# holandes22/etcd

Hardware: AMD Instinct MI355X
Metric: MsgAppResp applied/sec + commits advanced/sec, 1M raft groups×3, 1-8 GPUs (higher is better)
Workload: dtype u64

## Files before the change

etcd_amd/csrc/hipbatch.hip:

```cpp
#include <hip/hip_runtime.h>

#include <algorithm>
#include <cstdio>
#include <cstdlib>
#include <cstring>
#include <type_traits>
#include <utility>
#include <vector>

#include "hbmem.h"
#include "hipbatch_kernels.h"
#include "hipbatch_fast.h"
#include "hipbatch_elect.h"
#include "hipbatch_lead.h"
#include "hipbatch_wire.h"
#include "hipbatch_wire_in.h"
#include "hipbatch_wire_out.h"
#include "hipbatch_bin.h"

using namespace hb;

#define HB_CHECK(expr)                                                       \
  do {                                                                       \
    hipError_t _e = (expr);                                                  \
// ... 2777 lines not shown
  }
  if (threadIdx.x == 0) {
    a.bbase[nblk] = tot;
    decf_finish(a, tot);
  }
}
__global__ void __launch_bounds__(DEC_THREADS) k_decf_write(DecfArgs a, uint32_t nblk) {
  decf_write_block(a, blockIdx.x, a.bbase[blockIdx.x], a.bbase[nblk] <= a.ent_cap);
}
__global__ void __launch_bounds__(DEC_THREADS) k_decf_small(DecfArgs a, uint32_t nblk) {
  __shared__ uint64_t sh16[16];
  __shared__ uint64_t l_base[DEC_THREADS];
  uint64_t tot;
  l_base[threadIdx.x] = block_excl_scan64(threadIdx.x < nblk ? (uint64_t)a.bsum[threadIdx.x] : 0ull, sh16, &tot);
  __syncthreads();
  if (threadIdx.x == 0) decf_finish(a, tot);
  for (uint32_t b = 0; b < nblk; ++b) decf_write_block(a, b, l_base[b], tot <= a.ent_cap);
}

__global__ void __launch_bounds__(128) k_finish(uint64_t* shard, uint64_t* stats, uint64_t* accum) {
  const int map[ST_N + 1] = {HB_STAT_MSGS,  HB_STAT_APPRESP, HB_STAT_VOTERESP, HB_STAT_DROPPED, HB_STAT_COMMITS,
                             HB_STAT_WON,   HB_STAT_LOST,    HB_STAT_FAULTS,   HB_STAT_ENTRIES, HB_STAT_EVENTS};
  const uint32_t t = threadIdx.x, k = t / NSH;
  uint64_t v = 0;
  if (k <= ST_N) {
    v = shard[shard_at(k, t % NSH)];
    shard[shard_at(k, t % NSH)] = 0;
  }
#pragma unroll
  for (uint32_t d = 1; d < NSH; d <<= 1) v += __shfl_xor(v, d);
  if (k <= ST_N && t % NSH == 0) {
    stats[map[k]] = v;
    if (accum) accum[map[k]] += v;
  }
}

__global__ void k_load(DevState S, uint32_t first, uint32_t count, const hb_group* src) {
  const uint32_t i = blockIdx.x * blockDim.x + threadIdx.x;
  if (i >= count) return;
  const uint32_t g = first + i;
  const hb_group& r = src[i];
  S.term[g] = r.term;
  S.commit[g] = r.committed;
  S.first[g] = r.first_index;
  S.last[g] = r.last_index;
  S.tfirst[g] = r.term_first;
  S.tlast[g] = r.term_last;
  S.snap[g] = r.snap_index;
  uint64_t m = meta_make(r.state, r.n, r.self_slot, r.lead, r.vote, r.fault, r.votes_resp, r.votes_grant);
  if (r.term_last == r.last_index) m |= M_TL;
  if (r.self_slot < r.n && r.pr[r.self_slot].match == r.last_index && r.pr[r.self_slot].next == r.last_index + 1)
    m |= M_SM;
  if (r.commit_zero && r.committed != 0) m |= M_NC;
  S.meta[g] = m;
  S.elapsed[g] = 0;
  S.rpos[g] = 0;
  if (S.szx) {
    S.szlo[g] = r.last_index;
    *cum_at(S.szx[g], r.last_index) = 0;
  }
  S.trc[g] = 0;
  for (uint32_t s = 0; s < S.nmax; ++s) {
    const bool on = s < r.n;
    const size_t o = (size_t)s * S.G + g;
    S.match[o] = on ? r.pr[s].match : 0;
    S.next[o] = on ? r.pr[s].next : 0;
    S.pending[o] = on ? r.pr[s].pending_snapshot : 0;
    S.pm[o] = on ? pm_make(r.pr[s].state, r.pr[s].paused, r.pr[s].ins_start, r.pr[s].ins_count) : 0;
  }
}

__global__ void k_gather(DevState S, uint32_t first, uint32_t count, hb_group* dst) {
  const uint32_t i = blockIdx.x * blockDim.x + threadIdx.x;
  if (i >= count) return;
  const uint32_t g = first + i;
  hb_group r;
  memset(&r, 0, sizeof(r));
  const uint64_t m = S.meta[g];
  r.term = S.term[g];
  r.committed = S.commit[g];
  r.first_index = S.first[g];
  r.last_index = S.last[g];
  r.term_first = S.tfirst[g];
  r.term_last = (m & M_TL) ? r.last_index : S.tlast[g];
  r.snap_index = S.snap[g];
  r.state = m_state(m);
  r.n = m_n(m);
  r.self_slot = m_self(m);
  r.lead = m_lead(m);
  r.vote = m_vote(m);
  r.fault = m_fault(m);
  r.votes_resp = m_resp(m);
  r.votes_grant = m_grant(m);
  r.commit_zero = (m & M_NC) ? 1u : 0u;
  for (uint32_t s = 0; s < S.nmax && s < r.n; ++s) {
    const size_t o = (size_t)s * S.G + g;
    uint32_t p = S.pm[o];
    const bool kept = !((m & M_SM) && s == r.self_slot);
    r.pr[s].match = kept ? S.match[o] : r.last_index;
    r.pr[s].next = kept ? S.next[o] : r.last_index + 1;
    if (m & M_RS) rs_progress(m, s, r.last_index, r.term_first, &r.pr[s].match, &r.pr[s].next, &p);
    r.pr[s].state = pm_state(p);
    r.pr[s].paused = pm_paused(p);
    r.pr[s].ins_start = pm_start(p);
    r.pr[s].ins_count = pm_count(p);
    r.pr[s].pending_snapshot = pm_state(p) == HB_PR_SNAPSHOT ? S.pending[o] : 0;
  }
  dst[i] = r;
}

__global__ void k_set_bounds(DevState S, uint32_t count, const uint32_t* groups, const uint64_t* first,
                             const uint64_t* snap) {
  const uint32_t i = blockIdx.x * blockDim.x + threadIdx.x;
  if (i >= count) return;
  const uint32_t g = groups[i];
  S.first[g] = first[i];
  S.snap[g] = snap[i];
}

__global__ void k_load_runs(DevState S, uint32_t count, const uint32_t* groups, const uint32_t* n_runs,
                            const uint64_t* off, const uint64_t* runs) {
  const uint32_t i = blockIdx.x * blockDim.x + threadIdx.x;
  if (i >= count) return;
  const uint32_t g = groups[i], k = n_runs[i];
  uint64_t* R = lx_base(S.trx[g]);
  for (uint32_t j = 0; j < k; ++j) {
    R[2 * j] = runs[2 * (off[i] + j)];
    R[2 * j + 1] = runs[2 * (off[i] + j) + 1];
  }
  S.trc[g] = k;
}

__global__ void k_load_sizes(DevState S, uint32_t count, const uint32_t* groups, const uint32_t* n_sizes,
                             const uint64_t* off, const uint32_t* sizes) {
  const uint32_t i = blockIdx.x * blockDim.x + threadIdx.x;
  if (i >= count) return;
  const uint32_t g = groups[i], k = n_sizes[i];
  const uint64_t last = S.last[g], lo = last - k, x = S.szx[g];
  const uint32_t* z = sizes + off[i];
  uint64_t acc = 0;
  *cum_at(x, lo) = 0;
  for (uint32_t j = 1; j <= k; ++j) {
    acc += z[j - 1];
    *cum_at(x, lo + j) = acc;
  }
  S.szlo[g] = lo;
}

__global__ void k_regrow(DevState S, uint32_t count, const uint64_t* jobs) {
  const uint32_t i = blockIdx.x * blockDim.x + threadIdx.x;
  if (i >= count) return;
  const uint64_t* j = jobs + 4 * (size_t)i;
  const uint32_t g = (uint32_t)j[0], kind = (uint32_t)(j[0] >> 32);
  const uint64_t ox = j[1], nx = j[2];
  if (kind == 0) {
    const uint64_t lo = S.szlo[g], last = S.last[g];
    for (uint64_t k = lo; k <= last; ++k) *cum_at(nx, k) = *cum_at(ox, k);
    S.szx[g] = nx;
  } else {
    const uint64_t c = S.trc[g];
    const uint32_t n = (uint32_t)c, h = (uint32_t)(c >> 32);
// ... 1539 lines not shown
    const uint32_t gg = std::min(lists, GEN_GRID3 ? std::min(grid, GEN_GRID3) : grid);
    hipLaunchKernelGGL(k_apply<NMAX>, dim3(gg), dim3(PART), 0, h->stream, a);
  } else {
    hipLaunchKernelGGL(k_apply<NMAX>, dim3(std::min(lists, GEN_GRID ? std::min(grid, GEN_GRID) : grid)), dim3(PART), 0,
                       h->stream, a);
    hipLaunchKernelGGL(k_follow<NMAX>, dim3(FOLLOW_GRID), dim3(PART), 0, h->stream, a);
  }
  if (ev && full) (void)hipEventRecord(ev[4], h->stream);
}

}

extern "C" {

int hb_abi_version(void) { return HB_ABI_VERSION; }

const char* hb_strerror(int code) {
  switch (code) {
    case HB_OK: return "ok";
    case HB_EINVAL: return "invalid argument";
    case HB_ENOMEM: return "out of memory";
    case HB_EDEVICE: return "device error";
    case HB_EINVARIANT: return "device invariant violated";
    default: return "unknown error";
  }
}

int hb_create(int device, uint32_t capacity, uint32_t max_replicas, uint32_t max_inflight,
              uint64_t max_msg_size, uint64_t max_batch, hb_handle** out) {
  if (!out || capacity == 0 || max_replicas < 1 || max_replicas > HB_MAX_REPLICAS || max_inflight < 1 ||
      max_inflight > HB_MAX_INFLIGHT || max_batch >= (1ull << 31) || capacity > (1u << 24))
    return HB_EINVAL;
  int ndev = 0;
  if (hipGetDeviceCount(&ndev) != hipSuccess || device < 0 || device >= ndev) return HB_EDEVICE;
  DeviceGuard guard(device);
  hb_handle* h = new hb_handle();
  h->device = device;
  h->G = capacity;
  h->nmax = max_replicas <= 3 ? 3 : (max_replicas <= 5 ? 5 : 7);
  h->W = max_inflight;
  h->max_msg_size = max_msg_size;
  h->max_batch = max_batch;
  h->NB = (capacity + PART - 1) / PART;
  if (const char* e = getenv("HB_SMALL_STEP")) h->no_small = e[0] == '0';
  if (const char* e = getenv("HB_ROUTE_FUSE")) h->fuse = (uint32_t)atoi(e);
  if (const char* e = getenv("HB_STORM")) h->storm = atoi(e) == 0 ? 0u : 2u;
  if (const char* e = getenv("HB_FAST_STEADY")) h->steady = atoi(e) != 0;
  if (const char* e = getenv("HB_FAST_STEADY_COUNT")) h->steady_count = atoi(e) != 0;
  const size_t G = capacity, R = h->nmax;
  DevState& s = h->st;
  s.G = capacity;
  s.W = max_inflight;
  s.nmax = h->nmax;
  s.max_msg_size = max_msg_size;
  int rc = HB_OK;
#define ALLOC(ptr, count) \
  if (rc == HB_OK) rc = dalloc_t(h, &(ptr), (count))
  ALLOC(s.term, G);
  ALLOC(s.commit, G);
  ALLOC(s.first, G);
  ALLOC(s.last, G);
  ALLOC(s.tfirst, G);
  ALLOC(s.tlast, G);
  ALLOC(s.snap, G);
  ALLOC(s.meta, G);
  ALLOC(s.match, R * G);
  ALLOC(s.next, R * G);
  ALLOC(s.pending, R * G);
  ALLOC(s.pm, R * G);
  ALLOC(s.ring, R * (size_t)max_inflight * G);
  ALLOC(s.elapsed, G);
  ALLOC(s.rpos, G);
  ALLOC(s.tcfg, G);
  ALLOC(s.trx, G);
  ALLOC(s.trc, G);
  if (sz_on(max_msg_size)) {
    ALLOC(s.szx, G);
    ALLOC(s.szlo, G);
  }
  const size_t mb = max_batch ? max_batch : 1;
  auto nbk_for = [&](uint32_t sl) { return (capacity + (PART << sl) - 1) / (PART << sl); };
  auto passes_for = [&](uint32_t sl) {
    return (std::max<uint32_t>(ceil_log2(nbk_for(sl)), 1) + RDX_BITS - 1) / RDX_BITS;
  };
  const uint32_t sl_max = h->nmax <= 3 ? SIS_LOG_MAX3 : SIS_LOG_MAX;
  h->sis_log = sl_max;
  const uint32_t sl_min = route_rg_log(route_kmax(h->nmax)) - PART_LOG;
  while (h->sis_log > sl_min && passes_for(h->sis_log - 1) == passes_for(sl_max)) --h->sis_log;
  if (const char* e = getenv("HB_SIS_LOG")) {
    const int v = atoi(e);
    if (v >= (int)sl_min && v <= (int)sl_max) h->sis_log = (uint32_t)v;
  }
  h->NBK = nbk_for(h->sis_log);
  h->passes = passes_for(h->sis_log);
  h->bk_bits = std::max<uint32_t>(ceil_log2(h->NBK), 1);
  h->agrid = apply_grid_for(h->NBK, h->sis_log, h->NB);
  const size_t tiles_max = (mb + RDX_TILE - 1) / RDX_TILE;
  ALLOC(h->hist, (size_t)RDX_BINS * tiles_max);
  ALLOC(h->n_valid, 4);
  ALLOC(h->totals, RDX_BINS);
  if (h->passes == 1) {
    const size_t nhw = (tiles_max + HIST_TPB - 1) / HIST_TPB;
    h->sup_max = (uint32_t)((nhw + SB_HW - 1) / SB_HW);
    ALLOC(h->hagg, nhw * RDX_BINS);
    ALLOC(h->hsup, (size_t)SUP_BUFS * h->sup_max * RDX_BINS);
    if (rc == HB_OK && hipMemset(h->hsup, 0, (size_t)SUP_BUFS * h->sup_max * RDX_BINS * 4) != hipSuccess)
// ... 1284 lines not shown
int hb_stats_device(hb_handle* h, uint64_t** dev_stats) {
  if (!h || !dev_stats) return HB_EINVAL;
  *dev_stats = h->stats;
  return HB_OK;
}

int hb_stats(hb_handle* h, uint64_t* out) {
  if (!h || !out) return HB_EINVAL;
  DeviceGuard guard(h->device);
  HB_CHECK(hipMemcpyAsync(out, h->stats, HB_STAT_COUNT * 8, hipMemcpyDeviceToHost, h->stream));
  HB_CHECK(hipStreamSynchronize(h->stream));
  return HB_OK;
}

int hb_phase_ms(hb_handle* h, float* out, uint32_t* steps) {
  if (!h || !out) return HB_EINVAL;
  DeviceGuard guard(h->device);
  const uint32_t n = std::min<uint32_t>(h->prof_n, hb_handle::PROF_RING);
  if (steps) *steps = n;
  for (int i = 0; i < HB_PHASE_COUNT; ++i) out[i] = 0.f;
  if (n == 0) return HB_EINVAL;
  HB_CHECK(hipStreamSynchronize(h->prep));
  HB_CHECK(hipStreamSynchronize(h->stream));
  static const int span[HB_PHASE_COUNT][2] = {{0, 1}, {2, 3}, {3, 4}, {4, 5}};
  uint32_t nfull = 0;
  for (uint32_t k = 0; k < n; ++k) nfull += h->prof_full[k] ? 1u : 0u;
  for (uint32_t k = 0; k < n; ++k) {
    for (int i = 0; i < HB_PHASE_COUNT; ++i) {
      if (i != HB_PHASE_APPLY && !h->prof_full[k]) continue;
      float ms = 0.f;
      HB_CHECK(hipEventElapsedTime(&ms, h->ph[k][span[i][0]], h->ph[k][span[i][1]]));
      out[i] += ms / (float)(i == HB_PHASE_APPLY ? n : nfull);
    }
  }
  return HB_OK;
}

int hb_step_kernels(hb_handle* h, uint32_t* mask) {
  if (!h || !mask) return HB_EINVAL;
  *mask = h->kern;
  return HB_OK;
}

int hb_steady_waves(hb_handle* h, uint32_t* n) {
  if (!h || !n) return HB_EINVAL;
  *n = 0;
  if (!h->stepped || !h->steady_count) return HB_OK;
  DeviceGuard guard(h->device);
  HB_CHECK(hipStreamSynchronize(h->stream));
  HB_CHECK(hipMemcpy(n, h->set[h->cur].ctr + CTR_STEADY, 4, hipMemcpyDeviceToHost));
  return HB_OK;
}

int hb_phase_reset(hb_handle* h) {
  if (!h) return HB_EINVAL;
  h->prof_n = 0;
  return HB_OK;
}

int hb_set_stats_accum(hb_handle* h, uint64_t* dev_accum) {
  if (!h) return HB_EINVAL;
  h->stats_accum = dev_accum;
  return HB_OK;
}

int hb_set_input_stream(hb_handle* h, void* stream) {
  if (!h) return HB_EINVAL;
  h->in_stream = reinterpret_cast<hipStream_t>(stream);
  h->in_stream_set = true;
  return HB_OK;
}

int hb_stats_to(hb_handle* h, uint64_t* dev_dst) {
  if (!h || !dev_dst) return HB_EINVAL;
  DeviceGuard guard(h->device);
  HB_CHECK(hipMemcpyAsync(dev_dst, h->stats, HB_STAT_COUNT * 8, hipMemcpyDeviceToDevice, h->stream));
  return HB_OK;
}

int hb_alloc_pinned(size_t bytes, void** out) {
  if (!out) return HB_EINVAL;
  return hipHostMalloc(out, bytes ? bytes : 1, hipHostMallocDefault) == hipSuccess ? HB_OK : HB_ENOMEM;
}

int hb_free_pinned(void* p) { return hipHostFree(p) == hipSuccess ? HB_OK : HB_EDEVICE; }

}
```

etcd_amd/csrc/hipbatch_elect.h:

```cpp
#pragma once

#include "hipbatch_kernels.h"

namespace hb {

template <int NMAX>
struct ElectLane {
  DevState S;
  EvSink E;
  uint32_t g;
  uint64_t term, committed, last, tfirst, tlast, meta, meta0;
  uint64_t rlast;
  uint32_t dirty;
  uint32_t won, lost, nev;
  bool rst;
  bool sent;

  __device__ __forceinline__ uint32_t n() const { return m_n(meta); }
  __device__ __forceinline__ uint32_t state() const { return m_state(meta); }
  __device__ __forceinline__ uint32_t self() const { return m_self(meta); }
  __device__ __forceinline__ uint32_t lead() const { return m_lead(meta); }
  __device__ __forceinline__ uint32_t vote() const { return m_vote(meta); }
  __device__ __forceinline__ uint64_t soft() const {
    return (uint64_t)state() | ((uint64_t)lead() << 8) | ((uint64_t)vote() << 16);
  }
  __device__ __forceinline__ void set_field(int shift, uint64_t mask, uint64_t v) {
    meta = (meta & ~(mask << shift)) | ((v & mask) << shift);
    dirty |= D_META;
  }
  __device__ __forceinline__ void set_state(uint32_t v) { set_field(0, 3, v); }
  __device__ __forceinline__ void set_lead(uint32_t v) { set_field(9, 0xF, v); }
  __device__ __forceinline__ void set_vote(uint32_t v) { set_field(13, 0xF, v); }
  __device__ __forceinline__ void set_votes(uint32_t resp, uint32_t grant) {
    set_field(M_RESP_SHIFT, 0xFF, resp);
    set_field(M_GRANT_SHIFT, 0xFF, grant);
  }
  __device__ __forceinline__ void ev(uint32_t type, uint32_t to, uint32_t aux, uint64_t x) {
    emit_ev(E, g & (PART - 1), type, to, aux, x);
    nev++;
  }

  __device__ __forceinline__ void load() {
    term = S.term[g];
    committed = S.commit[g];
    last = S.last[g];
    tfirst = S.tfirst[g];
    tlast = S.tlast[g];
    meta0 = meta;
    if (meta & M_TL) tlast = last;
    dirty = 0;
    won = lost = nev = 0;
    rst = sent = false;
    rlast = 0;
  }

  __device__ __forceinline__ void store() {
    const uint32_t sf = self(), nn = n();
    const bool tl = tlast == last;
    const bool sm = rst ? sf < nn : (meta0 & M_SM) != 0;
    const bool leader = state() == HB_STATE_LEADER;
    const bool rs = rst && (leader ? (tfirst == rlast + 1 && (sent || nn <= 1)) : (rlast == last && !sent));
    const uint64_t m2 = (meta & ~(M_TL | M_SM | M_RS)) | (tl ? M_TL : 0ull) | (sm ? M_SM : 0ull) |
                        (rs ? M_RS : (rst ? 0ull : (meta & M_RS)));
    if (m2 != meta) {
      meta = m2;
      dirty |= D_META;
    }
    if (!tl && (meta0 & M_TL)) dirty |= D_TRUN;
    if (dirty & D_META) S.meta[g] = meta;
    if (dirty & D_TERM) S.term[g] = term;
    if (dirty & D_COMMIT) S.commit[g] = committed;
    if (dirty & D_LAST) S.last[g] = last;
    if (dirty & D_TRUN) {
      S.tfirst[g] = tfirst;
      S.tlast[g] = tlast;
    }
    if (dirty & D_ELAPSED) S.elapsed[g] = 0;
    if (rst && !rs) {
      const uint32_t peer_pm = pm_make(HB_PR_PROBE, sent ? 1u : 0u, 0, 0);
#pragma unroll
      for (int s = 0; s < NMAX; ++s) {
        if ((uint32_t)s < nn) {
          const bool me = (uint32_t)s == sf;
          S.match[(size_t)s * S.G + g] = me ? last : 0ull;
          S.next[(size_t)s * S.G + g] = me ? last + 1 : rlast + 1;
          S.pm[(size_t)s * S.G + g] = me ? pm_make(HB_PR_PROBE, 0, 0, 0) : peer_pm;
        }
      }
    }
  }

  __device__ __forceinline__ void reset(uint64_t t) {
    if (term != t) {
      if (tfirst != HB_NO_INDEX) tr_push(S, g, tfirst, term);
      term = t;
      set_vote(HB_REF_NONE);
      tfirst = HB_NO_INDEX;
      tlast = 0;
      dirty |= D_TERM | D_TRUN;
      ev(HB_EV_TERM, 0, 0, t);
    }
    set_lead(HB_REF_NONE);
    dirty |= D_ELAPSED;
    set_votes(0, 0);
    rst = true;
    sent = false;
    rlast = last;
  }
  __device__ __forceinline__ void transition(uint32_t kind, uint64_t t, uint32_t ld) {
    const uint64_t before = soft();
    reset(kind == HB_STATE_CANDIDATE ? term + 1 : (kind == HB_STATE_FOLLOWER ? t : term));
    set_lead(kind == HB_STATE_LEADER ? self() : (kind == HB_STATE_FOLLOWER ? ld : (uint32_t)HB_REF_NONE));
    if (kind == HB_STATE_CANDIDATE) set_vote(self());
    set_state(kind);
    if (soft() != before) ev(HB_EV_STATE, 0, 0, soft());
  }
// ... 86 lines not shown
```

etcd_amd/csrc/hipbatch_fast.h:

```cpp
#pragma once

#include "hipbatch_kernels.h"

namespace hb {

template <int NMAX>
struct FastLane {
  DevState S;
  EvSink E;
  uint32_t g;
  uint32_t arrival;
  uint64_t term, committed, first, last, tfirst, tlast;
  uint32_t mlo;
  uint64_t match[NMAX], next[NMAX], head[NMAX];
  uint32_t pm[NMAX];
  uint32_t dirty;
  uint32_t hv;
  static constexpr bool HEADS = NMAX <= 5;
  uint32_t nev;

  __device__ __forceinline__ uint32_t n() const { return (mlo >> 2) & 7; }
  __device__ __forceinline__ uint32_t state() const { return mlo & 3; }
  __device__ __forceinline__ uint32_t self() const { return (mlo >> 5) & 0xF; }
  __device__ __forceinline__ uint32_t faulted() const { return (mlo >> 17) & 0xF; }
  __device__ __forceinline__ uint64_t arrival_x() const {
    return arrival == 0xFFFFFFFFu ? HB_NO_INDEX : (uint64_t)arrival;
  }
  __device__ __forceinline__ void ev(uint32_t type, uint32_t to, uint32_t aux, uint64_t x) {
    emit_ev(E, g & (PART - 1), type, to, aux, x);
    nev++;
  }
  __device__ __forceinline__ void fault(uint32_t code) {
    if (faulted()) return;
    mlo = (mlo & ~(0xFu << 17)) | (code << 17);
    dirty |= D_META;
  }
  __device__ __forceinline__ uint64_t* ring_at(uint32_t s, uint32_t idx) const {
    return S.ring + ((size_t)s * S.W + idx) * S.G + g;
  }

  __device__ __forceinline__ void load() {
    load_head();
    load_rest();
  }
  __device__ __forceinline__ void load_head() {
    load_state_head();
    load_pm();
  }
  __device__ __forceinline__ void load_state_head() {
    term = at32(S.term, g);
    committed = at32(S.commit, g);
    first = at32(S.first, g);
    last = at32(S.last, g);
    tfirst = at32(S.tfirst, g);
  }
  __device__ __forceinline__ void load_pm() {
#pragma unroll
    for (int s = 0; s < NMAX; ++s) pm[s] = at32(S.pm, s * S.G + g);
  }
  __device__ __forceinline__ void load_rest() {
    tlast = (mlo & (uint32_t)M_TL) ? last : at32(S.tlast, g);
    const uint32_t sf = (mlo & (uint32_t)M_SM) ? self() : 0xFFu;
#pragma unroll
    for (int s = 0; s < NMAX; ++s) {
      match[s] = ((uint32_t)s == sf) ? last : at32(S.match, s * S.G + g);
      next[s] = ((uint32_t)s == sf) ? last + 1 : at32(S.next, s * S.G + g);
    }
    if (mlo & (uint32_t)M_RS) {
      const uint32_t nn = n();
#pragma unroll
      for (int s = 0; s < NMAX; ++s) {
        if ((uint32_t)s < nn) {
          uint64_t mt, nx;
          uint32_t p;
          rs_progress(mlo, (uint32_t)s, last, tfirst, &mt, &nx, &p);
          match[s] = mt;
          next[s] = nx;
          pm[s] = p;
        }
      }
    }
#pragma unroll
    for (int s = 0; s < NMAX; ++s) head[s] = (HEADS && pm_count(pm[s])) ? *ring_at(s, pm_start(pm[s])) : 0;
    hv = HEADS ? (1u << NMAX) - 1 : 0u;
    dirty = 0;
    if (mlo & (uint32_t)M_RS) {
      mlo &= ~(uint32_t)M_RS;
      dirty |= D_META;
#pragma unroll
      for (int s = 0; s < NMAX; ++s)
        if ((uint32_t)s < n()) dirty |= (1u << (D_SLOT0 + s)) | (1u << (D_PM0 + s));
    }
  }
  static constexpr uint32_t D_TFIRST = 1u << 5;
  static constexpr uint32_t D_PM0 = 16;
  __device__ __forceinline__ void store() {
    const bool tl = (mlo & (uint32_t)M_TL) && tlast == last;
    if ((mlo & (uint32_t)M_TL) && !tl) {
      mlo &= ~(uint32_t)M_TL;
      dirty |= D_META | D_TRUN;
    }
    uint32_t sf = 0xFFu;
    if (mlo & (uint32_t)M_SM) {
      const uint32_t s0 = self();
      bool ok = false;
#pragma unroll
      for (int s = 0; s < NMAX; ++s)
        if ((uint32_t)s == s0) ok = match[s] == last && next[s] == last + 1;
      if (ok) {
        sf = s0;
      } else {
        mlo &= ~(uint32_t)M_SM;
        dirty |= D_META | (1u << (D_SLOT0 + s0));
      }
    }
    if (dirty & D_META) at32(reinterpret_cast<uint32_t*>(S.meta), 2 * g) = mlo;
    if (dirty & D_COMMIT) at32(S.commit, g) = committed;
    if (dirty & D_LAST) at32(S.last, g) = last;
    if (dirty & D_TFIRST) at32(S.tfirst, g) = tfirst;
    if ((dirty & D_TRUN) && !tl) at32(S.tlast, g) = tlast;
#pragma unroll
    for (int s = 0; s < NMAX; ++s) {
      if ((dirty & (1u << (D_SLOT0 + s))) && (uint32_t)s != sf) {
        at32(S.match, s * S.G + g) = match[s];
        at32(S.next, s * S.G + g) = next[s];
      }
      if (dirty & (1u << (D_PM0 + s))) at32(S.pm, s * S.G + g) = pm[s];
    }
  }
  __device__ __forceinline__ void set_pm(int s, uint32_t v) {
    if (v != pm[s]) dirty |= 1u << (D_PM0 + s);
    pm[s] = v;
  }

  __device__ __forceinline__ bool is_paused(uint32_t p) const {
    const uint32_t st = pm_state(p);
    if (st == HB_PR_PROBE) return pm_paused(p) != 0;
    if (st == HB_PR_REPLICATE) return pm_count(p) == S.W;
    return true;
  }
  __device__ __forceinline__ void free_to(int s, uint64_t to, uint64_t nx0) {
    const uint32_t p = pm[s];
    const uint32_t cnt = pm_count(p);
    if (cnt == 0) return;
    uint32_t idx = pm_start(p);
    const uint32_t W = S.W;
    if (nx0 != 0 && to >= nx0 - 1) {
      idx += cnt;
      if (idx >= W) idx -= W;
      set_pm(s, pm_make(pm_state(p), pm_paused(p), idx, 0));
      return;
    }
    if (!((hv >> s) & 1u)) {
      head[s] = *ring_at(s, idx);
      hv |= 1u << s;
    }
    uint64_t v = head[s];
    if (to < v) return;
    uint32_t i = 0;
    while (true) {
      ++i;
      if (++idx >= W) idx -= W;
      if (i == cnt) break;
      v = *ring_at(s, idx);
      if (to < v) break;
    }
    set_pm(s, pm_make(pm_state(p), pm_paused(p), idx, cnt - i));
    head[s] = v;
  }
  __device__ __forceinline__ uint32_t lt_cur(uint64_t x) const { return (tfirst <= x && x <= tlast) ? 1u : 0u; }
  __device__ __forceinline__ bool term_eq(uint64_t i) const {
    if (i + 1 < first || i > last) return term == 0;
    return tfirst <= i && i <= tlast;
  }
  __device__ __forceinline__ bool maybe_commit() {
    uint64_t v[NMAX];
    const uint32_t nn = n();
#pragma unroll
// ... 212 lines not shown
      touch = true;
      f.pm = pm_make(HB_PR_REPLICATE, pm_paused(f.pm), pm_start(f.pm), c + 1);
    }
    ok = ok && f.next == last + 1;
    return x;
  }
  __device__ __forceinline__ void bcast(uint32_t W, uint64_t first, uint32_t j) {
    const uint64_t xa = send(fa, ring_a, add_a, touch_a, W, first);
    const uint64_t xb = send(fb, ring_b, add_b, touch_b, W, first);
    ok = ok && xa == xb;
    if (jfirst == 0) {
      jfirst = j;
      xfirst = xa;
    }
    evm |= 1u << j;
    ltm |= lt_cur(xa) << j;
  }
  __device__ __forceinline__ bool maybe_commit(uint64_t term, uint64_t first, uint32_t j) {
    const uint64_t mx = umax64(smatch, fa.match), mn = umin64(smatch, fa.match);
    const uint64_t mci = umax64(mn, umin64(mx, fb.match));
    const bool teq = (mci + 1 < first || mci > last) ? term == 0 : (tfirst <= mci && mci <= tlast);
    const bool up = mci > committed && teq;
    ok = ok && !(up && (last < mci || (evm & EVM_COMMIT) != 0));
    if (up) {
      committed = mci;
      evm |= 1u << j;
    }
    return up;
  }
  __device__ __forceinline__ void ack(uint32_t info, uint64_t mterm, uint64_t index, uint64_t term, uint32_t W,
                                      uint64_t first, uint32_t t) {
    const uint32_t type = info & 0xF, from = (info >> 4) & 0xF;
    const bool reject = (info >> 8) & 1u;
    ok = ok && type == HB_MSG_APP_RESP && !reject && (mterm == 0 || mterm == term) && (from == sa || from == sb);
    const bool isa = from == sa;
    const uint64_t am = fa.match, an = fa.next, bm = fb.match, bn = fb.next;
    const uint32_t ap = fa.pm, bp = fb.pm;
    const uint64_t m0 = isa ? am : bm, nx0 = isa ? an : bn;
    const uint32_t p0 = isa ? ap : bp;
    const uint32_t c = pm_count(p0);
    ok = ok && c != W && m0 < index && index <= last && nx0 != 0 && index >= nx0 - 1;
    const uint64_t nx = umax64(nx0, index + 1);
    uint32_t idx = pm_start(p0) + c;
    if (c != 0 && idx >= W) idx -= W;
    const uint32_t p = pm_make(HB_PR_REPLICATE, 0, idx, 0);
    fa.match = isa ? index : am;
    fa.next = isa ? nx : an;
    fa.pm = isa ? p : ap;
    touch_a = touch_a || isa;
    fb.match = isa ? bm : index;
    fb.next = isa ? bn : nx;
    fb.pm = isa ? bp : p;
    touch_b = touch_b || !isa;
    if (maybe_commit(term, first, EW_P + 2 * t)) bcast(W, first, EW_P + 2 * t + 1);
  }

  __device__ __forceinline__ void plan(const FastLane<3>& L, uint32_t prop_k, uint32_t cnt,
                                       const uint32_t (&s_info)[2], const uint32_t (&s_orig)[2],
                                       const uint64_t (&s_term)[2], const uint64_t (&s_index)[2]) {
    const uint32_t W = L.S.W;
    last = L.last;
    committed = L.committed;
    tfirst = L.tfirst;
    tlast = L.tlast;
    sf = L.self();
    sa = sf == 0 ? 1u : 0u;
    sb = sf == 2 ? 1u : 2u;
    const uint64_t m0 = L.match[0], m1 = L.match[1], m2 = L.match[2];
    const uint64_t n0 = L.next[0], n1 = L.next[1], n2 = L.next[2];
    const uint32_t p0 = L.pm[0], p1 = L.pm[1], p2 = L.pm[2];
    smatch = sf == 0 ? m0 : (sf == 1 ? m1 : m2);
    snext = sf == 0 ? n0 : (sf == 1 ? n1 : n2);
    spm = spm0 = sf == 0 ? p0 : (sf == 1 ? p1 : p2);
    fa.match = sf == 0 ? m1 : m0;
    fa.next = sf == 0 ? n1 : n0;
    fa.pm = pa0 = sf == 0 ? p1 : p0;
    fb.match = sf == 2 ? m1 : m2;
    fb.next = sf == 2 ? n1 : n2;
    fb.pm = pb0 = sf == 2 ? p1 : p2;
    add_a = add_b = touch_a = touch_b = false;
    ring_a = ring_b = 0;
    evm = ltm = jfirst = 0;
    xfirst = 0;
    prop = d_tfirst = false;
    ok = L.n() == 3 && sf < 3 && !(L.mlo & (uint32_t)M_RS) && L.S.max_msg_size == HB_NO_LIMIT && cnt <= 2 &&
         pm_state(fa.pm) == HB_PR_REPLICATE && pm_state(fb.pm) == HB_PR_REPLICATE;
    if (prop_k) {
      prop = true;
      const uint64_t old = last;
      last += prop_k;
      if (tfirst == HB_NO_INDEX) {
        tfirst = old + 1;
        d_tfirst = true;
      }
      tlast = last;
      evm |= 1u;
      if (smatch < last) {
        smatch = last;
        spm &= ~PM_PAUSED;
      }
      if (snext < last + 1) snext = last + 1;
      maybe_commit(L.term, L.first, 1);
      bcast(W, L.first, 2);
    }
    const uint32_t ia = s_info[0], ib = s_info[1], oa = s_orig[0], ob = s_orig[1];
    const uint64_t ta = s_term[0], tb = s_term[1], xa = s_index[0], xb = s_index[1];
    const bool sw = cnt == 2 && ob < oa;
    const uint32_t i0 = sw ? ib : ia, i1 = sw ? ia : ib;
    const uint64_t t0 = sw ? tb : ta, t1 = sw ? ta : tb;
    const uint64_t x0 = sw ? xb : xa, x1 = sw ? xa : xb;
    if (cnt == 2) ok = ok && ((i0 ^ i1) & 0xF0u) != 0;
    if (cnt >= 1) ack(i0, t0, x0, L.term, W, L.first, 0);
    if (cnt >= 2) ack(i1, t1, x1, L.term, W, L.first, 1);
    ok = ok && ((last | xfirst) >> 40) == 0;
  }
  __device__ __forceinline__ uint32_t nev() const { return __popc(evm) + __popc(evm & EVM_BCAST); }
  __device__ __forceinline__ uint64_t word(uint32_t j, uint32_t lane) const {
    if (j == 0) return evc_word(HB_EV_LAST, 0, 0, lane, last, false);
    if ((EVM_COMMIT >> j) & 1u) return evc_word(HB_EV_COMMIT, 0, 0, lane, committed, false);
    return evc_word(EVC_BCAST, (1u << sa) | (1u << sb), (ltm >> j) & 1u, lane, j == jfirst ? xfirst : last, false);
  }

  __device__ __forceinline__ void commit(const FastLane<3>& L) const {
    const DevState& S = L.S;
    const uint32_t g = L.g;
    if (committed != L.committed) at32(S.commit, g) = committed;
    if (prop) {
      at32(S.last, g) = last;
      if (d_tfirst) at32(S.tfirst, g) = tfirst;
      if (!(L.mlo & (uint32_t)M_TL)) at32(S.tlast, g) = tlast;
      if (!(L.mlo & (uint32_t)M_SM)) {
        at32(S.match, sf * S.G + g) = smatch;
        at32(S.next, sf * S.G + g) = snext;
      }
    }
    if (spm != spm0) at32(S.pm, sf * S.G + g) = spm;
    if (touch_a) {
      at32(S.match, sa * S.G + g) = fa.match;
      at32(S.next, sa * S.G + g) = fa.next;
    }
    if (fa.pm != pa0) at32(S.pm, sa * S.G + g) = fa.pm;
    if (add_a) *L.ring_at(sa, ring_a) = last;
    if (touch_b) {
      at32(S.match, sb * S.G + g) = fb.match;
      at32(S.next, sb * S.G + g) = fb.next;
    }
    if (fb.pm != pb0) at32(S.pm, sb * S.G + g) = fb.pm;
    if (add_b) *L.ring_at(sb, ring_b) = last;
  }
};

}
```

etcd_amd/csrc/hipbatch_kernels.h:

```cpp
#pragma once

#include <hip/hip_runtime.h>
#include <stdint.h>

#include "../../include/hipbatch.h"

namespace hb {

#ifndef HB_PART_LOG
#define HB_PART_LOG 8
#endif
constexpr int PART_LOG = HB_PART_LOG;
constexpr uint32_t PART = 1u << PART_LOG;
#ifndef HB_APPLY_WAVES3
#define HB_APPLY_WAVES3 3
#endif
constexpr uint32_t CHUNK = 4 * PART;

constexpr int M_GRANT_SHIFT = 32;
constexpr int M_RESP_SHIFT = 40;
__host__ __device__ inline uint64_t meta_make(uint32_t state, uint32_t n, uint32_t self, uint32_t lead,
                                              uint32_t vote, uint32_t fault, uint32_t resp, uint32_t grant) {
  return (uint64_t)(state & 3) | ((uint64_t)(n & 7) << 2) | ((uint64_t)(self & 0xF) << 5) |
         ((uint64_t)(lead & 0xF) << 9) | ((uint64_t)(vote & 0xF) << 13) | ((uint64_t)(fault & 0xF) << 17) |
         ((uint64_t)(resp & 0xFF) << M_RESP_SHIFT) | ((uint64_t)(grant & 0xFF) << M_GRANT_SHIFT);
}
constexpr uint64_t M_TL = 1ull << 21;
constexpr uint64_t M_SM = 1ull << 22;
constexpr uint64_t M_RS = 1ull << 23;
constexpr uint64_t M_NC = 1ull << 24;
__host__ __device__ inline uint32_t m_state(uint64_t m) { return (uint32_t)(m & 3); }
__host__ __device__ inline uint32_t m_n(uint64_t m) { return (uint32_t)((m >> 2) & 7); }
__host__ __device__ inline uint32_t m_self(uint64_t m) { return (uint32_t)((m >> 5) & 0xF); }
__host__ __device__ inline uint32_t m_lead(uint64_t m) { return (uint32_t)((m >> 9) & 0xF); }
__host__ __device__ inline uint32_t m_vote(uint64_t m) { return (uint32_t)((m >> 13) & 0xF); }
__host__ __device__ inline uint32_t m_fault(uint64_t m) { return (uint32_t)((m >> 17) & 0xF); }
__host__ __device__ inline uint32_t m_resp(uint64_t m) { return (uint32_t)((m >> M_RESP_SHIFT) & 0xFF); }
__host__ __device__ inline uint32_t m_grant(uint64_t m) { return (uint32_t)((m >> M_GRANT_SHIFT) & 0xFF); }

__host__ __device__ inline uint32_t pm_make(uint32_t st, uint32_t paused, uint32_t start, uint32_t count) {
  return (st & 3) | ((paused & 1) << 2) | ((start & 0x3FF) << 3) | ((count & 0x7FF) << 13);
}
__host__ __device__ inline uint32_t pm_state(uint32_t p) { return p & 3; }
__host__ __device__ inline uint32_t pm_paused(uint32_t p) { return (p >> 2) & 1; }
__host__ __device__ inline uint32_t pm_start(uint32_t p) { return (p >> 3) & 0x3FF; }
__host__ __device__ inline uint32_t pm_count(uint32_t p) { return (p >> 13) & 0x7FF; }
constexpr uint32_t PM_PAUSED = 1u << 2;

__device__ __forceinline__ void rs_progress(uint64_t m, uint32_t s, uint64_t last, uint64_t tfirst, uint64_t* match,
                                            uint64_t* next, uint32_t* pm) {
  const bool leader = m_state(m) == HB_STATE_LEADER;
  const uint64_t rl = leader ? tfirst - 1 : last;
  const bool me = s == m_self(m);
  *match = me ? last : 0ull;
  *next = me ? last + 1 : rl + 1;
  *pm = pm_make(HB_PR_PROBE, (!me && leader) ? 1u : 0u, 0, 0);
}

struct DevState {
  uint32_t G;
  uint32_t W;
  uint32_t nmax;
  uint32_t pad;
  uint64_t max_msg_size;
  uint64_t* term;
  uint64_t* commit;
  uint64_t* first;
  uint64_t* last;
  uint64_t* tfirst;
  uint64_t* tlast;
  uint64_t* snap;
  uint64_t* meta;
  uint64_t* match;
  uint64_t* next;
  uint64_t* pending;
  uint32_t* pm;
  uint64_t* ring;
  uint32_t* elapsed;
  uint32_t* rpos;
  uint32_t* tcfg;
  const uint64_t* rnd;
  uint64_t nrnd;
  uint64_t* szx;
  uint64_t* szlo;
  const uint32_t* edesc;
  const uint64_t* eoff;
  const uint64_t* peoff;
  uint64_t* trx;
  uint64_t* trc;
  const uint64_t* bcommit;
  const uint64_t* eterm;
  uint64_t n_ent;
  uint64_t bn;
};

template <class T>
__device__ __forceinline__ T& at32(T* base, uint32_t i) {
  return *reinterpret_cast<T*>(reinterpret_cast<char*>(base) + i * (uint32_t)sizeof(T));
}
template <class T>
__device__ __forceinline__ const T& at32(const T* base, uint32_t i) {
  return *reinterpret_cast<const T*>(reinterpret_cast<const char*>(base) + i * (uint32_t)sizeof(T));
}

constexpr uint64_t LX_TAG = 0x3F;
__host__ __device__ inline uint64_t lx_word(uint64_t addr, uint32_t log2cap) { return addr | log2cap; }
__device__ __forceinline__ uint64_t* lx_base(uint64_t x) { return reinterpret_cast<uint64_t*>(x & ~LX_TAG); }
__device__ __forceinline__ uint64_t lx_cap(uint64_t x) { return 1ull << (x & LX_TAG); }

__host__ __device__ inline bool sz_on(uint64_t max_msg_size) { return max_msg_size != 0 && max_msg_size != HB_NO_LIMIT; }
__device__ __forceinline__ uint64_t sov(uint64_t x) { return x ? (uint64_t)(70 - __clzll(x)) / 7 : 1; }
__device__ __forceinline__ uint64_t ent_size(uint32_t desc, uint64_t term, uint64_t index) {
  uint64_t n = 1 + sov((desc >> 30) & 1u) + 1 + sov(term) + 1 + sov(index);
  if (desc >> 31) {
    const uint64_t l = desc & HB_ENT_MAX_DATA;
    n += 1 + l + sov(l);
// ... 206 lines not shown
  __device__ __forceinline__ void set_votes(uint32_t resp, uint32_t grant) {
    set_field(M_RESP_SHIFT, 0xFF, resp);
    set_field(M_GRANT_SHIFT, 0xFF, grant);
  }

  __device__ __forceinline__ uint64_t arrival_x() const {
    return arrival == 0xFFFFFFFFu ? HB_NO_INDEX : (uint64_t)arrival;
  }
  __device__ __forceinline__ void ev(uint32_t type, uint32_t to, uint32_t aux, uint64_t x) {
    emit_ev(E, g & (PART - 1), type, to, aux, x);
    nev++;
  }
  __device__ __forceinline__ void fault(uint32_t code) {
    if (faulted()) return;
    set_field(17, 0xF, code);
  }

  __device__ __forceinline__ uint64_t* ring_at(uint32_t s, uint32_t idx) const {
    return S.ring + ((size_t)s * S.W + idx) * S.G + g;
  }
  __device__ __forceinline__ Pr get(uint32_t s) const {
    Pr p;
    p.match = match[s];
    p.next = next[s];
    p.pm = pm[s];
    p.head = head[s];
    return p;
  }
  __device__ __forceinline__ void put(uint32_t s, const Pr& p) {
    match[s] = p.match;
    next[s] = p.next;
    pm[s] = p.pm;
    head[s] = p.head;
    dirty |= 1u << (D_SLOT0 + s);
  }

  __device__ __forceinline__ void load_all() {
    load_group();
    load_progress();
  }
  __device__ __forceinline__ void load_group() {
    term = S.term[g];
    committed = S.commit[g];
    first = S.first[g];
    last = S.last[g];
    tfirst = S.tfirst[g];
    tlast = S.tlast[g];
    meta0 = meta;
    if (meta & M_TL) tlast = last;
    dirty = 0;
    prog = false;
  }
  __device__ __forceinline__ void load_progress() {
#pragma unroll
    for (int s = 0; s < NMAX; ++s) {
      match[s] = S.match[(size_t)s * S.G + g];
      next[s] = S.next[(size_t)s * S.G + g];
      pm[s] = S.pm[(size_t)s * S.G + g];
    }
    if (meta & M_RS) {
      const uint32_t nn = n();
#pragma unroll
      for (int s = 0; s < NMAX; ++s) {
        if ((uint32_t)s < nn) {
          uint64_t mt, nx;
          uint32_t p;
          rs_progress(meta, (uint32_t)s, last, tfirst, &mt, &nx, &p);
          match[s] = mt;
          next[s] = nx;
          pm[s] = p;
          dirty |= 1u << (D_SLOT0 + s);
        }
      }
      meta &= ~M_RS;
      dirty |= D_META;
    }
#pragma unroll
    for (int s = 0; s < NMAX; ++s) head[s] = pm_count(pm[s]) ? *ring_at(s, pm_start(pm[s])) : 0;
    if (meta0 & M_SM) {
      const uint32_t sf = m_self(meta0);
#pragma unroll
      for (int s = 0; s < NMAX; ++s) {
        if ((uint32_t)s == sf) {
          match[s] = last;
          next[s] = last + 1;
        }
      }
    }
    prog = true;
  }

  __device__ __forceinline__ void store() {
    if (dirty & D_FIRST) S.first[g] = first;
    {
      const uint32_t sf = self(), nn = n();
      const bool tl = tlast == last;
      bool sm = (meta0 & M_SM) != 0;
      if (prog) {
        sm = false;
#pragma unroll
        for (int s = 0; s < NMAX; ++s)
          if ((uint32_t)s == sf && (uint32_t)s < nn) sm = match[s] == last && next[s] == last + 1;
      }
      const uint64_t m2 = (meta & ~(M_TL | M_SM)) | (tl ? M_TL : 0ull) | (sm ? M_SM : 0ull);
      if (m2 != meta) {
        meta = m2;
        dirty |= D_META;
      }
      if (!tl && (meta0 & M_TL)) dirty |= D_TRUN;
      if (!sm && (meta0 & M_SM) && sf < (uint32_t)NMAX) dirty |= 1u << (D_SLOT0 + sf);
    }
    if (dirty & D_META) S.meta[g] = meta;
    if (dirty & D_TERM) S.term[g] = term;
    if (dirty & D_COMMIT) S.commit[g] = committed;
    if (dirty & D_LAST) S.last[g] = last;
    if (dirty & D_TRUN) {
      S.tfirst[g] = tfirst;
      S.tlast[g] = tlast;
    }
    if (dirty & D_ELAPSED) S.elapsed[g] = 0;
#pragma unroll
    for (int s = 0; s < NMAX; ++s) {
      if (dirty & (1u << (D_SLOT0 + s))) {
        S.match[(size_t)s * S.G + g] = match[s];
        S.next[(size_t)s * S.G + g] = next[s];
        S.pm[(size_t)s * S.G + g] = pm[s];
      }
    }
  }

  __device__ __forceinline__ bool is_paused(uint32_t p) const {
    const uint32_t st = pm_state(p);
    if (st == HB_PR_PROBE) return pm_paused(p) != 0;
    if (st == HB_PR_REPLICATE) return pm_count(p) == S.W;
    return true;
  }
  __device__ __forceinline__ void become_probe(uint32_t s, Pr& p) const {
    if (pm_state(p.pm) == HB_PR_SNAPSHOT) {
      const uint64_t pending = S.pending[(size_t)s * S.G + g];
      p.pm = pm_make(HB_PR_PROBE, 0, 0, 0);
      p.next = umax64(p.match + 1, pending + 1);
    } else {
      p.pm = pm_make(HB_PR_PROBE, 0, 0, 0);
      p.next = p.match + 1;
    }
  }
  __device__ __forceinline__ void become_replicate(Pr& p) const {
    p.pm = pm_make(HB_PR_REPLICATE, 0, 0, 0);
    p.next = p.match + 1;
  }
  __device__ __forceinline__ bool maybe_update(Pr& p, uint64_t nidx) const {
    bool updated = false;
    if (p.match < nidx) {
      p.match = nidx;
      updated = true;
      p.pm &= ~PM_PAUSED;
    }
    if (p.next < nidx + 1) p.next = nidx + 1;
    return updated;
  }
  __device__ __forceinline__ bool maybe_decr_to(Pr& p, uint64_t rejected, uint64_t lasthint) const {
    if (pm_state(p.pm) == HB_PR_REPLICATE) {
      if (rejected <= p.match) return false;
      p.next = p.match + 1;
      return true;
    }
    if (p.next - 1 != rejected) return false;
    p.next = umin64(rejected, lasthint + 1);
    if (p.next < 1) p.next = 1;
    p.pm &= ~PM_PAUSED;
    return true;
  }
  __device__ __forceinline__ void free_to(uint32_t s, Pr& p, uint64_t to) const {
    const uint32_t cnt = pm_count(p.pm);
    if (cnt == 0) return;
    uint64_t v = p.head;
    if (to < v) return;
    uint32_t idx = pm_start(p.pm);
// ... 539 lines not shown
```

etcd_amd/hipbatch.py:

```python
import ctypes as C
import os

import numpy as np

from . import abi

_HERE = os.path.dirname(os.path.abspath(__file__))
LIB_PATH = os.environ.get("HB_LIB", os.path.join(_HERE, "libhipbatch.so"))
_lib = None


class HipBatchError(RuntimeError):
    def __init__(self, fn, code):
        self.code = code
        super().__init__(f"{fn} failed: {code} ({_strerror(code)})")


def _strerror(code):
    try:
        return lib().hb_strerror(code).decode()
    except Exception:
        return "?"


# ... 401 lines not shown
            if total <= cap:
                break
            cap = total
        words = np.ctypeslib.as_array((C.c_uint64 * max(total, 1)).from_address(w))[:total].copy()
        counts = np.ctypeslib.as_array((C.c_uint32 * nc).from_address(cnt)).copy()
        return words, counts

    @staticmethod
    def expand_words(words, counts):
        L = lib()
        w = np.ascontiguousarray(words, dtype=np.uint64)
        c = np.ascontiguousarray(counts, dtype=np.uint32)
        n = C.c_uint64()
        _check("hb_expand_event_words", L.hb_expand_event_words(w.ctypes.data, len(w), c.ctypes.data, len(c), None,
                                                                0, C.byref(n)))
        out = np.zeros(max(n.value, 1), dtype=abi.EVENT_DTYPE)
        _check("hb_expand_event_words", L.hb_expand_event_words(w.ctypes.data, len(w), c.ctypes.data, len(c),
                                                                out.ctypes.data, len(out), C.byref(n)))
        return out[: n.value]

    def stats(self):
        out = np.zeros(abi.HB_STAT_COUNT, dtype=np.uint64)
        _check("hb_stats", lib().hb_stats(self.h, out.ctypes.data))
        return out

    def stats_device_ptr(self):
        p = C.c_void_p()
        _check("hb_stats_device", lib().hb_stats_device(self.h, C.byref(p)))
        return p.value

    def stats_to(self, dev_ptr):
        _check("hb_stats_to", lib().hb_stats_to(self.h, C.c_void_p(_ptr(dev_ptr) if not isinstance(dev_ptr, int)
                                                                   else dev_ptr)))

    def set_stats_accum(self, dev_ptr):
        p = None if dev_ptr is None else (dev_ptr if isinstance(dev_ptr, int) else _ptr(dev_ptr))
        _check("hb_set_stats_accum", lib().hb_set_stats_accum(self.h, C.c_void_p(p)))

    def phase_reset(self):
        _check("hb_phase_reset", lib().hb_phase_reset(self.h))

    def step_kernels(self):
        m = C.c_uint32()
        _check("hb_step_kernels", lib().hb_step_kernels(self.h, C.byref(m)))
        return int(m.value)

    def steady_waves(self):
        f = lib().hb_steady_waves
        f.restype, f.argtypes = C.c_int, [C.c_void_p, C.POINTER(C.c_uint32)]
        n = C.c_uint32()
        _check("hb_steady_waves", f(self.h, C.byref(n)))
        return int(n.value)

    def phase_ms(self):
        out = np.zeros(abi.HB_PHASE_COUNT, dtype=np.float32)
        n = C.c_uint32()
        _check("hb_phase_ms", lib().hb_phase_ms(self.h, out.ctypes.data, C.byref(n)))
        return out, n.value
```

include/hipbatch.h:

```cpp
#ifndef HIPBATCH_H_
#define HIPBATCH_H_

#include <stddef.h>
#include <stdint.h>

#ifdef __cplusplus
extern "C" {
#endif

#define HB_ABI_VERSION 8

#define HB_OK          0
#define HB_EINVAL     -1
#define HB_ENOMEM     -2
#define HB_EDEVICE    -3
#define HB_EINVARIANT -4

#define HB_MAX_REPLICAS   7
#define HB_MAX_INFLIGHT   1024
#define HB_NO_LIMIT       UINT64_MAX
#define HB_NO_INDEX       UINT64_MAX
#define HB_SIZE_RING_MIN  16
#define HB_TERM_RING_MIN  8

// ... 205 lines not shown
typedef struct hb_out_batch {
  uint32_t* group;
  uint32_t* info;
  uint64_t* to;
  uint64_t* term;
  uint64_t* log_term;
  uint64_t* index;
  uint64_t* commit;
  uint64_t* hint;
} hb_out_batch;
#define HB_EGRESS_ON    1
#define HB_EGRESS_VOTES 2
#define HB_EGRESS_APPS  4
int  hb_set_egress(hb_handle* h, int on);
int  hb_egress_mode(hb_handle* h);
int  hb_egress_caps(void);
#define HB_OUT_HOST     0x400u
#define HB_OUT_ENTS     0x800u
int  hb_egress(hb_handle* h, uint64_t self_id, const hb_out_batch* out, uint64_t cap, uint64_t* count);
#define HB_WIRE_SPLICE 0x80
int  hb_encode(hb_handle* h, const hb_out_batch* in, uint64_t cap, const uint64_t* n_dev, uint64_t self_id,
               uint8_t* bytes, uint64_t bytes_cap, uint64_t* off , uint8_t* status ,
               uint64_t* total);

#define HB_EGRESS_MAX_PEERS 255
int  hb_set_egress_peers(hb_handle* h, const uint64_t* ids, uint32_t n);
int  hb_egress_bin(hb_handle* h, const hb_out_batch* in, uint64_t cap, const uint64_t* n_dev,
                   const hb_out_batch* out, uint32_t* src, uint64_t* bin_off);
int  hb_peer_spans(hb_handle* h, const uint64_t* off, const uint64_t* bin_off, uint64_t* span);

int  hb_step(hb_handle* h, const hb_batch* b, uint32_t flags);

#define HB_EVW_BCAST 12
#define HB_EVW_VBCAST 0
#define HB_EVW_CONT  15
int  hb_events_device(hb_handle* h, const uint64_t** base, const uint64_t** chunk_off,
                      const uint32_t** counts, uint32_t* n_chunks);
int  hb_copy_events(hb_handle* h, hb_event* out, uint64_t cap, uint64_t* n);
int  hb_events_to_host(hb_handle* h, uint64_t* words, uint64_t cap, uint32_t* counts, uint64_t* total);
int  hb_event_words_chunks(hb_handle* h, uint32_t* n_chunks, uint32_t* groups_per_chunk);
int  hb_expand_event_words(const uint64_t* words, uint64_t n_words, const uint32_t* counts, uint32_t n_chunks,
                           hb_event* out, uint64_t cap, uint64_t* n_out);
int  hb_stats_device(hb_handle* h, uint64_t** dev_stats);
int  hb_stats(hb_handle* h, uint64_t* out);
int  hb_stats_to(hb_handle* h, uint64_t* dev_dst );
int  hb_set_stats_accum(hb_handle* h, uint64_t* dev_accum);
int  hb_phase_ms(hb_handle* h, float* out , uint32_t* steps);
int  hb_phase_reset(hb_handle* h);
#define HB_KERN_ROUTE_FAST 1u
#define HB_KERN_ROUTE_ELECT 2u
int  hb_step_kernels(hb_handle* h, uint32_t* mask);
int  hb_steady_waves(hb_handle* h, uint32_t* n);

int  hb_alloc_pinned(size_t bytes, void** out);
int  hb_free_pinned(void* p);

#ifdef __cplusplus
}
#endif
#endif
```

Baseline: 23.43 billion.

## Encode all-caught-up next indices as a meta bit to skip next-array traffic

Adds an M_NX meta flag marking leader groups (up to 3 replicas) where every peer's next equals last+1. While the flag is set, the fast, elect and general kernels derive next from last instead of reading it, and skip storing the per-slot next arrays. When the condition breaks, they write back all slots. The aim is to cut global memory reads and writes of next in the steady-state MsgAppResp path. The cost is extra per-lane flag logic, a correctness risk in the flag transitions, and an added ring-accounting tweak (add_a/add_b) plus a debug counter API.

```diff
diff --git a/etcd_amd/csrc/hipbatch.hip b/etcd_amd/csrc/hipbatch.hip
--- a/etcd_amd/csrc/hipbatch.hip
+++ b/etcd_amd/csrc/hipbatch.hip
@@ -2853,6 +2853,9 @@
   if (r.self_slot < r.n && r.pr[r.self_slot].match == r.last_index && r.pr[r.self_slot].next == r.last_index + 1)
     m |= M_SM;
   if (r.commit_zero && r.committed != 0) m |= M_NC;
+  bool nx = S.lazy_next != 0 && r.state == HB_STATE_LEADER && r.n != 0 && r.n <= S.nmax;
+  for (uint32_t s = 0; s < S.nmax && s < r.n; ++s) nx = nx && r.pr[s].next == r.last_index + 1;
+  if (nx) m |= M_NX;
   S.meta[g] = m;
   S.elapsed[g] = 0;
   S.rpos[g] = 0;
@@ -2865,7 +2868,7 @@
     const bool on = s < r.n;
     const size_t o = (size_t)s * S.G + g;
     S.match[o] = on ? r.pr[s].match : 0;
-    S.next[o] = on ? r.pr[s].next : 0;
+    if (!(nx && on)) S.next[o] = on ? r.pr[s].next : 0;
     S.pending[o] = on ? r.pr[s].pending_snapshot : 0;
     S.pm[o] = on ? pm_make(r.pr[s].state, r.pr[s].paused, r.pr[s].ins_start, r.pr[s].ins_count) : 0;
   }
@@ -2899,7 +2902,7 @@
     uint32_t p = S.pm[o];
     const bool kept = !((m & M_SM) && s == r.self_slot);
     r.pr[s].match = kept ? S.match[o] : r.last_index;
-    r.pr[s].next = kept ? S.next[o] : r.last_index + 1;
+    r.pr[s].next = (kept && !(m & M_NX)) ? S.next[o] : r.last_index + 1;
     if (m & M_RS) rs_progress(m, s, r.last_index, r.term_first, &r.pr[s].match, &r.pr[s].next, &p);
     r.pr[s].state = pm_state(p);
     r.pr[s].paused = pm_paused(p);
@@ -2908,6 +2911,13 @@
     r.pr[s].pending_snapshot = pm_state(p) == HB_PR_SNAPSHOT ? S.pending[o] : 0;
   }
   dst[i] = r;
+}
+
+__global__ void k_count_lazy_next(DevState S, uint32_t* out) {
+  const uint32_t g = blockIdx.x * blockDim.x + threadIdx.x;
+  const uint64_t m = g < S.G ? S.meta[g] : 0ull;
+  const uint64_t b = __ballot(m_n(m) != 0 && (m & M_NX) != 0);
+  if ((threadIdx.x & 63) == 0 && b) atomicAdd(out, (uint32_t)__popcll(b));
 }
 
 __global__ void k_set_bounds(DevState S, uint32_t count, const uint32_t* groups, const uint64_t* first,
@@ -4553,6 +4563,8 @@
   s.G = capacity;
   s.W = max_inflight;
   s.nmax = h->nmax;
+  s.lazy_next = h->nmax <= 3 ? 1u : 0u;
+  if (const char* e = getenv("HB_LAZY_NEXT")) s.lazy_next = (h->nmax <= 3 && atoi(e) != 0) ? 1u : 0u;
   s.max_msg_size = max_msg_size;
   int rc = HB_OK;
 #define ALLOC(ptr, count) \
@@ -5943,6 +5955,19 @@
   return HB_OK;
 }
 
+int hb_lazy_next_groups(hb_handle* h, uint32_t* n) {
+  if (!h || !n) return HB_EINVAL;
+  *n = 0;
+  DeviceGuard guard(h->device);
+  Dev<uint32_t> d;
+  if (const int rc = d.reserve(1)) return rc;
+  HB_CHECK(hipMemsetAsync(d.get(), 0, 4, h->stream));
+  hipLaunchKernelGGL(k_count_lazy_next, dim3((h->G + 255) / 256), dim3(256), 0, h->stream, h->st, d.get());
+  HB_CHECK(hipMemcpyAsync(n, d.get(), 4, hipMemcpyDeviceToHost, h->stream));
+  HB_CHECK(hipStreamSynchronize(h->stream));
+  return HB_OK;
+}
+
 int hb_phase_reset(hb_handle* h) {
   if (!h) return HB_EINVAL;
   h->prof_n = 0;
diff --git a/etcd_amd/csrc/hipbatch_elect.h b/etcd_amd/csrc/hipbatch_elect.h
--- a/etcd_amd/csrc/hipbatch_elect.h
+++ b/etcd_amd/csrc/hipbatch_elect.h
@@ -60,8 +60,8 @@
     const bool sm = rst ? sf < nn : (meta0 & M_SM) != 0;
     const bool leader = state() == HB_STATE_LEADER;
     const bool rs = rst && (leader ? (tfirst == rlast + 1 && (sent || nn <= 1)) : (rlast == last && !sent));
-    const uint64_t m2 = (meta & ~(M_TL | M_SM | M_RS)) | (tl ? M_TL : 0ull) | (sm ? M_SM : 0ull) |
-                        (rs ? M_RS : (rst ? 0ull : (meta & M_RS)));
+    const uint64_t m2 = (meta & ~(M_TL | M_SM | M_RS | (rst ? M_NX : 0ull))) | (tl ? M_TL : 0ull) |
+                        (sm ? M_SM : 0ull) | (rs ? M_RS : (rst ? 0ull : (meta & M_RS)));
     if (m2 != meta) {
       meta = m2;
       dirty |= D_META;
diff --git a/etcd_amd/csrc/hipbatch_fast.h b/etcd_amd/csrc/hipbatch_fast.h
--- a/etcd_amd/csrc/hipbatch_fast.h
+++ b/etcd_amd/csrc/hipbatch_fast.h
@@ -61,10 +61,11 @@
   __device__ __forceinline__ void load_rest() {
     tlast = (mlo & (uint32_t)M_TL) ? last : at32(S.tlast, g);
     const uint32_t sf = (mlo & (uint32_t)M_SM) ? self() : 0xFFu;
+    const bool nxl = NMAX <= 3 && (mlo & (uint32_t)M_NX) != 0;
 #pragma unroll
     for (int s = 0; s < NMAX; ++s) {
       match[s] = ((uint32_t)s == sf) ? last : at32(S.match, s * S.G + g);
-      next[s] = ((uint32_t)s == sf) ? last + 1 : at32(S.next, s * S.G + g);
+      next[s] = ((uint32_t)s == sf || nxl) ? last + 1 : at32(S.next, s * S.G + g);
     }
     if (mlo & (uint32_t)M_RS) {
       const uint32_t nn = n();
@@ -114,6 +115,23 @@
         dirty |= D_META | (1u << (D_SLOT0 + s0));
       }
     }
+    bool nx = false;
+    if constexpr (NMAX <= 3) {
+      const uint32_t nn = n();
+      nx = S.lazy_next != 0 && state() == HB_STATE_LEADER && nn != 0;
+#pragma unroll
+      for (int s = 0; s < NMAX; ++s)
+        if ((uint32_t)s < nn) nx = nx && next[s] == last + 1;
+      if (nx != ((mlo & (uint32_t)M_NX) != 0)) {
+        if (!nx) {
+#pragma unroll
+          for (int s = 0; s < NMAX; ++s)
+            if ((uint32_t)s < nn) dirty |= 1u << (D_SLOT0 + s);
+        }
+        mlo ^= (uint32_t)M_NX;
+        dirty |= D_META;
+      }
+    }
     if (dirty & D_META) at32(reinterpret_cast<uint32_t*>(S.meta), 2 * g) = mlo;
     if (dirty & D_COMMIT) at32(S.commit, g) = committed;
     if (dirty & D_LAST) at32(S.last, g) = last;
@@ -123,7 +141,7 @@
     for (int s = 0; s < NMAX; ++s) {
       if ((dirty & (1u << (D_SLOT0 + s))) && (uint32_t)s != sf) {
         at32(S.match, s * S.G + g) = match[s];
-        at32(S.next, s * S.G + g) = next[s];
+        if (!nx) at32(S.next, s * S.G + g) = next[s];
       }
       if (dirty & (1u << (D_PM0 + s))) at32(S.pm, s * S.G + g) = pm[s];
     }
@@ -442,6 +460,8 @@
     fb.next = isa ? bn : nx;
     fb.pm = isa ? bp : p;
     touch_b = touch_b || !isa;
+    add_a = add_a && !isa;
+    add_b = add_b && isa;
     if (maybe_commit(term, first, EW_P + 2 * t)) bcast(W, first, EW_P + 2 * t + 1);
   }
 
@@ -514,27 +534,25 @@
   __device__ __forceinline__ void commit(const FastLane<3>& L) const {
     const DevState& S = L.S;
     const uint32_t g = L.g;
+    const bool nx0 = (L.mlo & (uint32_t)M_NX) != 0;
+    const bool nx = S.lazy_next != 0 && snext == last + 1 && fa.next == last + 1 && fb.next == last + 1;
+    const bool all = nx0 && !nx;
+    if (nx != nx0) at32(reinterpret_cast<uint32_t*>(S.meta), 2 * g) = L.mlo ^ (uint32_t)M_NX;
     if (committed != L.committed) at32(S.commit, g) = committed;
     if (prop) {
       at32(S.last, g) = last;
       if (d_tfirst) at32(S.tfirst, g) = tfirst;
       if (!(L.mlo & (uint32_t)M_TL)) at32(S.tlast, g) = tlast;
-      if (!(L.mlo & (uint32_t)M_SM)) {
-        at32(S.match, sf * S.G + g) = smatch;
-        at32(S.next, sf * S.G + g) = snext;
-      }
-    }
+      if (!(L.mlo & (uint32_t)M_SM)) at32(S.match, sf * S.G + g) = smatch;
+    }
+    if (!(L.mlo & (uint32_t)M_SM) && !nx && (prop || all)) at32(S.next, sf * S.G + g) = snext;
     if (spm != spm0) at32(S.pm, sf * S.G + g) = spm;
-    if (touch_a) {
-      at32(S.match, sa * S.G + g) = fa.match;
-      at32(S.next, sa * S.G + g) = fa.next;
-    }
+    if (touch_a) at32(S.match, sa * S.G + g) = fa.match;
+    if (!nx && (touch_a || all)) at32(S.next, sa * S.G + g) = fa.next;
     if (fa.pm != pa0) at32(S.pm, sa * S.G + g) = fa.pm;
     if (add_a) *L.ring_at(sa, ring_a) = last;
-    if (touch_b) {
-      at32(S.match, sb * S.G + g) = fb.match;
-      at32(S.next, sb * S.G + g) = fb.next;
-    }
+    if (touch_b) at32(S.match, sb * S.G + g) = fb.match;
+    if (!nx && (touch_b || all)) at32(S.next, sb * S.G + g) = fb.next;
     if (fb.pm != pb0) at32(S.pm, sb * S.G + g) = fb.pm;
     if (add_b) *L.ring_at(sb, ring_b) = last;
   }
diff --git a/etcd_amd/csrc/hipbatch_kernels.h b/etcd_amd/csrc/hipbatch_kernels.h
--- a/etcd_amd/csrc/hipbatch_kernels.h
+++ b/etcd_amd/csrc/hipbatch_kernels.h
@@ -29,6 +29,7 @@
 constexpr uint64_t M_SM = 1ull << 22;
 constexpr uint64_t M_RS = 1ull << 23;
 constexpr uint64_t M_NC = 1ull << 24;
+constexpr uint64_t M_NX = 1ull << 25;
 __host__ __device__ inline uint32_t m_state(uint64_t m) { return (uint32_t)(m & 3); }
 __host__ __device__ inline uint32_t m_n(uint64_t m) { return (uint32_t)((m >> 2) & 7); }
 __host__ __device__ inline uint32_t m_self(uint64_t m) { return (uint32_t)((m >> 5) & 0xF); }
@@ -61,7 +62,7 @@
   uint32_t G;
   uint32_t W;
   uint32_t nmax;
-  uint32_t pad;
+  uint32_t lazy_next;
   uint64_t max_msg_size;
   uint64_t* term;
   uint64_t* commit;
@@ -374,10 +375,11 @@
     prog = false;
   }
   __device__ __forceinline__ void load_progress() {
+    const bool nxl = NMAX <= 3 && (meta0 & M_NX) != 0;
 #pragma unroll
     for (int s = 0; s < NMAX; ++s) {
       match[s] = S.match[(size_t)s * S.G + g];
-      next[s] = S.next[(size_t)s * S.G + g];
+      next[s] = nxl ? ((uint32_t)s < n() ? last + 1 : 0ull) : S.next[(size_t)s * S.G + g];
       pm[s] = S.pm[(size_t)s * S.G + g];
     }
     if (meta & M_RS) {
@@ -414,6 +416,7 @@
 
   __device__ __forceinline__ void store() {
     if (dirty & D_FIRST) S.first[g] = first;
+    bool nx;
     {
       const uint32_t sf = self(), nn = n();
       const bool tl = tlast == last;
@@ -424,13 +427,26 @@
         for (int s = 0; s < NMAX; ++s)
           if ((uint32_t)s == sf && (uint32_t)s < nn) sm = match[s] == last && next[s] == last + 1;
       }
-      const uint64_t m2 = (meta & ~(M_TL | M_SM)) | (tl ? M_TL : 0ull) | (sm ? M_SM : 0ull);
+      nx = NMAX <= 3 && (meta0 & M_NX) != 0;
+      if (NMAX <= 3 && prog) {
+        nx = S.lazy_next != 0 && state() == HB_STATE_LEADER && nn != 0 && !(meta & M_RS);
+#pragma unroll
+        for (int s = 0; s < NMAX; ++s)
+          if ((uint32_t)s < nn) nx = nx && next[s] == last + 1;
+      }
+      const uint64_t m2 =
+          (meta & ~(M_TL | M_SM | M_NX)) | (tl ? M_TL : 0ull) | (sm ? M_SM : 0ull) | (nx ? M_NX : 0ull);
       if (m2 != meta) {
         meta = m2;
         dirty |= D_META;
       }
       if (!tl && (meta0 & M_TL)) dirty |= D_TRUN;
       if (!sm && (meta0 & M_SM) && sf < (uint32_t)NMAX) dirty |= 1u << (D_SLOT0 + sf);
+      if (!nx && (meta0 & M_NX)) {
+#pragma unroll
+        for (int s = 0; s < NMAX; ++s)
+          if ((uint32_t)s < nn) dirty |= 1u << (D_SLOT0 + s);
+      }
     }
     if (dirty & D_META) S.meta[g] = meta;
     if (dirty & D_TERM) S.term[g] = term;
@@ -445,7 +461,7 @@
     for (int s = 0; s < NMAX; ++s) {
       if (dirty & (1u << (D_SLOT0 + s))) {
         S.match[(size_t)s * S.G + g] = match[s];
-        S.next[(size_t)s * S.G + g] = next[s];
+        if (!nx) S.next[(size_t)s * S.G + g] = next[s];
         S.pm[(size_t)s * S.G + g] = pm[s];
       }
     }
diff --git a/etcd_amd/hipbatch.py b/etcd_amd/hipbatch.py
--- a/etcd_amd/hipbatch.py
+++ b/etcd_amd/hipbatch.py
@@ -477,6 +477,13 @@
         _check("hb_steady_waves", f(self.h, C.byref(n)))
         return int(n.value)
 
+    def lazy_next_groups(self):
+        f = lib().hb_lazy_next_groups
+        f.restype, f.argtypes = C.c_int, [C.c_void_p, C.POINTER(C.c_uint32)]
+        n = C.c_uint32()
+        _check("hb_lazy_next_groups", f(self.h, C.byref(n)))
+        return int(n.value)
+
     def phase_ms(self):
         out = np.zeros(abi.HB_PHASE_COUNT, dtype=np.float32)
         n = C.c_uint32()
diff --git a/include/hipbatch.h b/include/hipbatch.h
--- a/include/hipbatch.h
+++ b/include/hipbatch.h
@@ -281,6 +281,8 @@
 int  hb_step_kernels(hb_handle* h, uint32_t* mask);
 int  hb_steady_waves(hb_handle* h, uint32_t* n);
 
+int  hb_lazy_next_groups(hb_handle* h, uint32_t* n);
+
 int  hb_alloc_pinned(size_t bytes, void** out);
 int  hb_free_pinned(void* p);
 
```

Result: faster. 25.06 billion, median of 6 (+7.0%).
